# traveller59/spconv

Hardware: NVIDIA H100
Metric: active-voxels/sec fwd+bwd SubMConv3d 3^3 C=64 (higher is better)
Workload: dtype fp16

## Files before the change

### spconv_b200/csrc/common.cuh

```cuda
#pragma once
#include <cuda_runtime.h>
#include <cuda_fp16.h>
#include <cuda_bf16.h>
#include <stdint.h>
#include <stdio.h>
#include <string.h>
#include <stdarg.h>
#include <type_traits>

#include "../../include/spconv_b200.h"

namespace spx {

void set_error(const char *fmt, ...);
void count_launch(int n = 1);
void set_family(int f);
int sm_count();
int current_device();

struct RuntimeCfg {
    int force_simt = 0, force_tc = 0;
    bool tf32_dgrad_fma = false;
    bool tf32_wgrad_fma = false;
};
RuntimeCfg &runtime_cfg();

bool func_configured(const void *fn, int dev);

#define SPX_CHECK_CUDA(expr)                                                              \
    do {                                                                                  \
        cudaError_t _e = (expr);                                                          \
        if (_e != cudaSuccess) {                                                          \
            (void)cudaGetLastError();                                                     \
            spx::set_error("%s failed: %s (%s:%d)", #expr, cudaGetErrorString(_e),        \
                           __FILE__, __LINE__);                                           \
            return 1;                                                                     \
        }                                                                                 \
    } while (0)

#define SPX_CHECK_LAUNCH(name)                                                            \
    do {                                                                                  \
        cudaError_t _e = cudaGetLastError();                                              \
        if (_e != cudaSuccess) {                                                          \
            spx::set_error("launch of %s failed: %s (%s:%d)", name,                       \
                           cudaGetErrorString(_e), __FILE__, __LINE__);                   \
            return 1;                                                                     \
        }                                                                                 \
        spx::count_launch();                                                              \
    } while (0)

#define SPX_REQUIRE(cond, ...)                                                            \
    do {                                                                                  \
        if (!(cond)) {                                                                    \
            spx::set_error(__VA_ARGS__);                                                  \
            return 2;                                                                     \
        }                                                                                 \
    } while (0)

static inline size_t align_up(size_t x, size_t a) { return (x + a - 1) / a * a; }
static inline int64_t div_up64(int64_t a, int64_t b) { return (a + b - 1) / b; }

struct WorkspaceCarver {
    char *base;
    size_t off = 0, cap;
    WorkspaceCarver(void *p, size_t bytes) : base((char *)p), cap(bytes) {}
    template <typename T> T *take(size_t n) {
        off = align_up(off, 256);
        T *r = (T *)(base + off);
        off += n * sizeof(T);
        return r;
    }
    bool ok() const { return off <= cap; }
};

__host__ __device__ static inline int dtype_bytes(int dt) {
    switch (dt) {
        case SPX_F32: return 4;
        case SPX_F16: return 2;
        case SPX_BF16: return 2;
        case SPX_I8: return 1;
    }
    return 0;
}

#ifdef __CUDACC__

template <typename T> __device__ __forceinline__ float to_float(T v);
template <> __device__ __forceinline__ float to_float<float>(float v) { return v; }
template <> __device__ __forceinline__ float to_float<__half>(__half v) { return __half2float(v); }
template <> __device__ __forceinline__ float to_float<__nv_bfloat16>(__nv_bfloat16 v) { return __bfloat162float(v); }
template <> __device__ __forceinline__ float to_float<int8_t>(int8_t v) { return (float)v; }

template <typename T> __device__ __forceinline__ T from_float(float v);
template <> __device__ __forceinline__ float from_float<float>(float v) { return v; }
template <> __device__ __forceinline__ __half from_float<__half>(float v) { return __float2half_rn(v); }
template <> __device__ __forceinline__ __nv_bfloat16 from_float<__nv_bfloat16>(float v) { return __float2bfloat16_rn(v); }

__device__ __forceinline__ float apply_act(float v, int act, float alpha) {
    switch (act) {
        case SPX_ACT_RELU: return v > 0.f ? v : 0.f;
        case SPX_ACT_SIGMOID: return 1.f / (1.f + __expf(-v));
        case SPX_ACT_LEAKY_RELU: return v >= 0.f ? v : v * alpha;
        default: return v;
    }
}

__device__ __forceinline__ uint32_t smem_u32(const void *p) {
    return (uint32_t)__cvta_generic_to_shared(p);
}

__device__ __forceinline__ void mbar_init(uint64_t *bar, uint32_t count) {
    asm volatile("mbarrier.init.shared::cta.b64 [%0], %1;" ::"r"(smem_u32(bar)), "r"(count) : "memory");
}
__device__ __forceinline__ void mbar_fence_init() {
    asm volatile("fence.mbarrier_init.release.cluster;" ::: "memory");
}
__device__ __forceinline__ void mbar_arrive(uint64_t *bar) {
    asm volatile("{\n\t.reg .b64 st;\n\tmbarrier.arrive.shared::cta.b64 st, [%0];\n\t}" ::"r"(smem_u32(bar)) : "memory");
}
__device__ __forceinline__ void mbar_arrive_expect_tx(uint64_t *bar, uint32_t bytes) {
    asm volatile("{\n\t.reg .b64 st;\n\tmbarrier.arrive.expect_tx.shared::cta.b64 st, [%0], %1;\n\t}" ::"r"(smem_u32(bar)), "r"(bytes) : "memory");
}
__device__ __forceinline__ bool mbar_try_wait(uint64_t *bar, uint32_t parity) {
    uint32_t ok;
    asm volatile(
        "{\n\t.reg .pred p;\n\t"
        "mbarrier.try_wait.parity.shared::cta.b64 p, [%1], %2;\n\t"
        "selp.u32 %0, 1, 0, p;\n\t}"
        : "=r"(ok) : "r"(smem_u32(bar)), "r"(parity) : "memory");
    return ok != 0;
}
__device__ __forceinline__ void mbar_wait(uint64_t *bar, uint32_t parity) {
    if (mbar_try_wait(bar, parity)) return;
    const long long t0 = clock64();
    uint32_t spins = 0;
    while (!mbar_try_wait(bar, parity)) {
        if ((++spins & 0x3FFFu) == 0u && clock64() - t0 > 4000000000ll) {
            printf("spconv_b200: mbarrier wait timed out (block %d thread %d bar 0x%x parity %u)\n",
                   (int)blockIdx.x, (int)threadIdx.x, smem_u32(bar), parity);
            __trap();
        }
// ... 69 lines not shown
```

### spconv_b200/csrc/rulebook.cu

```cuda
#include "common.cuh"
#include "gemm.cuh"
#include "hash.cuh"
#include "rank.cuh"
#include <cub/cub.cuh>

namespace spx {
size_t radix_argsort_workspace_bytes(int64_t n);
int radix_argsort_pair(uint32_t *mask0, int32_t *argsort0, int64_t n0, uint32_t *mask1, int32_t *argsort1, int64_t n1,
                       int key_bits, void *ws0, size_t ws0_bytes, void *ws1, size_t ws1_bytes, cudaStream_t stream);
}

namespace spx {

struct Geom {
    int ndim, batch, kv;
    int in_dims[SPX_MAX_NDIM], out_dims[SPX_MAX_NDIM], ksize[SPX_MAX_NDIM];
    int stride[SPX_MAX_NDIM], padding[SPX_MAX_NDIM], dilation[SPX_MAX_NDIM];
    int transposed;
};

static Geom make_geom(const spx_conv_geometry *g, bool subm) {
    Geom r;
    memset(&r, 0, sizeof(r));
    r.ndim = g->ndim;
    r.batch = g->batch_size;
    r.kv = 1;
    r.transposed = g->transposed;
    for (int a = 0; a < g->ndim; ++a) {
        r.in_dims[a] = g->in_dims[a];
        r.ksize[a] = g->ksize[a];
        r.dilation[a] = g->dilation[a];
        r.kv *= g->ksize[a];
        if (subm) {
            r.out_dims[a] = g->in_dims[a];
            r.stride[a] = 1;
            r.padding[a] = (g->ksize[a] / 2) * g->dilation[a];
        } else {
            r.out_dims[a] = g->out_dims[a];
            r.stride[a] = g->stride[a];
            r.padding[a] = g->padding[a];
        }
    }
    return r;
}

static bool needs_i64(const Geom &g, const int *dims) {
    double v = (double)g.batch;
    for (int a = 0; a < g.ndim; ++a) v *= (double)dims[a];
    return v >= 2147483647.0;
}

__device__ __forceinline__ void load_coord(const int32_t *indices, int64_t i, int ndim, int (&c)[SPX_MAX_NDIM + 1]) {
    if (ndim == 3) {
        int4 v = __ldg(reinterpret_cast<const int4 *>(indices) + i);
        c[0] = v.x; c[1] = v.y; c[2] = v.z; c[3] = v.w;
    } else {
        const int32_t *p = indices + i * (ndim + 1);
#pragma unroll
        for (int a = 0; a <= SPX_MAX_NDIM; ++a) if (a <= ndim) c[a] = __ldg(p + a);
    }
}

__device__ __forceinline__ int64_t linear_key(const int (&c)[SPX_MAX_NDIM + 1], const int *dims, int ndim) {
    int64_t k = c[0];
#pragma unroll
    for (int a = 0; a < SPX_MAX_NDIM; ++a) if (a < ndim) k = k * dims[a] + c[a + 1];
    return k;
}

__device__ __forceinline__ void offset_taps(int k, const int *ksize, int ndim, int (&r)[SPX_MAX_NDIM]) {
#pragma unroll
    for (int a = SPX_MAX_NDIM - 1; a >= 0; --a) if (a < ndim) { r[a] = k % ksize[a]; k /= ksize[a]; }
}

template <typename Table>
__global__ void subm_insert_kernel(Table table, Geom g, const int32_t *__restrict__ indices, int64_t N) {
    int64_t i = blockIdx.x * (int64_t)blockDim.x + threadIdx.x;
    if (i >= N) return;
    int c[SPX_MAX_NDIM + 1];
    load_coord(indices, i, g.ndim, c);
    table.insert_min(linear_key(c, g.in_dims, g.ndim), (int32_t)i);
}

template <typename Table>
__global__ void subm_probe_kernel(Table table, Geom g, const int32_t *__restrict__ indices, int64_t N,
                                  int32_t *__restrict__ pair_fwd, int32_t *__restrict__ pair_bwd,
                                  uint32_t *__restrict__ mask, int words) {
    int64_t o = blockIdx.x * (int64_t)blockDim.x + threadIdx.x;
    if (o >= N) return;
    int c[SPX_MAX_NDIM + 1];
    load_coord(indices, o, g.ndim, c);
    const int kv = g.kv;
    uint32_t mword = 0;
    int r[SPX_MAX_NDIM] = {0, 0, 0, 0};
    for (int k = 0; k < kv; ++k) {
        int32_t found = -1;
        if (k == kv / 2) {
            found = (int32_t)o;
        } else {
            int q[SPX_MAX_NDIM + 1];
            q[0] = c[0];
            bool valid = c[0] >= 0 && c[0] < g.batch;
#pragma unroll
            for (int a = 0; a < SPX_MAX_NDIM; ++a) {
                if (a < g.ndim) {
                    q[a + 1] = c[a + 1] - g.padding[a] + r[a] * g.dilation[a];
                    valid = valid && q[a + 1] >= 0 && q[a + 1] < g.in_dims[a];
                }
            }
            if (valid) {
                int32_t v;
                if (table.find_slot(linear_key(q, g.in_dims, g.ndim), v) >= 0) found = v;
            }
        }
        pair_fwd[(int64_t)k * N + o] = found;
        if (pair_bwd) pair_bwd[(int64_t)(kv - 1 - k) * N + o] = found;
        if (found >= 0) mword |= 1u << (k & 31);
        if (mask && ((k & 31) == 31 || k == kv - 1)) {
            mask[o * words + (k >> 5)] = mword;
            mword = 0;
        }
#pragma unroll
        for (int a = SPX_MAX_NDIM - 1; a >= 0; --a) {
            if (a < g.ndim) {
                if (++r[a] < g.ksize[a]) break;
                r[a] = 0;
            }
        }
    }
}

constexpr int K3_VOX = 128;
constexpr int K3_PER_LANE = K3_VOX / 32;
__global__ void __launch_bounds__(27 * 32, 2)
subm_probe_k3_kernel(Table32 table, Geom g, const int32_t *__restrict__ indices, int64_t N,
                     int32_t *__restrict__ pair_fwd, int32_t *__restrict__ pair_bwd,
                     uint32_t *__restrict__ mask, int32_t *__restrict__ row_table) {
    __shared__ uint32_t hit_col[27][K3_PER_LANE];
    __shared__ int32_t row_stage[K3_VOX][27];
    const int lane = threadIdx.x & 31;
    const int k = threadIdx.x >> 5;
    const int rz = k / 9, ry = (k / 3) % 3, rx = k % 3;
    const int64_t vbase = blockIdx.x * (int64_t)K3_VOX;
    const int D0 = g.in_dims[0], D1 = g.in_dims[1], D2 = g.in_dims[2];
    const int oz = (rz - 1) * g.dilation[0], oy = (ry - 1) * g.dilation[1], ox = (rx - 1) * g.dilation[2];
    int4 c[K3_PER_LANE];
#pragma unroll
    for (int j = 0; j < K3_PER_LANE; ++j) {
        const int64_t o = vbase + j * 32 + lane;
        c[j] = o < N ? __ldg(reinterpret_cast<const int4 *>(indices) + o) : make_int4(-1, 0, 0, 0);
    }
    uint32_t key[K3_PER_LANE], h[K3_PER_LANE];
    unsigned long long cur[K3_PER_LANE];
    uint32_t pending = 0;
#pragma unroll
    for (int j = 0; j < K3_PER_LANE; ++j) {
        const int qz = c[j].y + oz, qy = c[j].z + oy, qx = c[j].w + ox;
        const bool valid = k != 13 && c[j].x >= 0 && c[j].x < g.batch && qz >= 0 && qz < D0 && qy >= 0 && qy < D1 &&
                           qx >= 0 && qx < D2;
        key[j] = (uint32_t)(((c[j].x * D0 + qz) * D1 + qy) * D2 + qx);
        h[j] = mix32(key[j]) & table.cap_mask;
        cur[j] = valid ? __ldg(&table.slots[h[j]]) : Table32::EMPTY;
    }
#pragma unroll
    for (int j = 0; j < K3_PER_LANE; ++j)
        if (cur[j] != Table32::EMPTY && (uint32_t)(cur[j] >> 32) != key[j]) pending |= 1u << j;
    while (pending) {
#pragma unroll
        for (int j = 0; j < K3_PER_LANE; ++j)
            if (pending & (1u << j)) { h[j] = (h[j] + 1) & table.cap_mask; cur[j] = __ldg(&table.slots[h[j]]); }
#pragma unroll
        for (int j = 0; j < K3_PER_LANE; ++j)
            if ((pending & (1u << j)) && (cur[j] == Table32::EMPTY || (uint32_t)(cur[j] >> 32) == key[j]))
                pending &= ~(1u << j);
    }
#pragma unroll
    for (int j = 0; j < K3_PER_LANE; ++j) {
        const int64_t o = vbase + j * 32 + lane;
        int32_t found = cur[j] != Table32::EMPTY ? (int32_t)(uint32_t)cur[j] : -1;
        if (k == 13 && o < N) found = (int32_t)o;
        if (o < N) {
            pair_fwd[(int64_t)k * N + o] = found;
            if (pair_bwd) pair_bwd[(int64_t)(26 - k) * N + o] = found;
        }
        const uint32_t hits = __ballot_sync(0xffffffffu, found >= 0);
        if (lane == 0) hit_col[k][j] = hits;
        row_stage[j * 32 + lane][k] = found;
    }
    __syncthreads();
    if (mask && threadIdx.x < K3_VOX && vbase + threadIdx.x < N) {
        const int v = threadIdx.x;
        uint32_t m = 0;
#pragma unroll
        for (int kk = 0; kk < 27; ++kk) m |= ((hit_col[kk][v >> 5] >> (v & 31)) & 1u) << kk;
        mask[vbase + v] = m;
    }
    if (row_table) {
        for (int e = threadIdx.x; e < K3_VOX * 32; e += 27 * 32) {
            const int v = e >> 5, kk = e & 31;
            if (vbase + v < N) row_table[(vbase + v) * 32 + kk] = kk < 27 ? row_stage[v][kk] : -1;
        }
    }
}

__device__ __forceinline__ bool conv_out_coord(const Geom &g, const int (&c)[SPX_MAX_NDIM + 1],
                                               const int (&r)[SPX_MAX_NDIM], int (&o)[SPX_MAX_NDIM + 1]) {
    bool valid = c[0] >= 0 && c[0] < g.batch;
    o[0] = c[0];
#pragma unroll
    for (int a = 0; a < SPX_MAX_NDIM; ++a) {
        if (a < g.ndim) {
            if (g.transposed) {
                o[a + 1] = c[a + 1] * g.stride[a] - g.padding[a] + r[a] * g.dilation[a];
                valid = valid && o[a + 1] >= 0 && o[a + 1] < g.out_dims[a];
            } else {
                int h = c[a + 1] + g.padding[a] - r[a] * g.dilation[a];
                o[a + 1] = h / g.stride[a];
                valid = valid && o[a + 1] >= 0 && o[a + 1] < g.out_dims[a] && (h % g.stride[a] == 0);
            }
        }
    }
    return valid;
}

struct Taps3 { int r0, r1, r2; };
__device__ __forceinline__ Taps3 block_taps3(const Geom &g, int k) {
    Taps3 t;
    t.r2 = k % g.ksize[2]; k /= g.ksize[2];
    t.r1 = k % g.ksize[1]; k /= g.ksize[1];
    t.r0 = k;
    return t;
}
__device__ __forceinline__ bool axis_out(int c, int pad, int r, int dil, int stride, int odim, int &o) {
    const int h = c + pad - r * dil;
    if (h < 0) return false;
    if (stride == 1) o = h;
    else if (stride == 2) { if (h & 1) return false; o = h >> 1; }
    else { o = h / stride; if (o * stride != h) return false; }
    return o < odim;
}
__device__ __forceinline__ bool conv3_out_key(const Geom &g, const int4 c, const Taps3 &t, int64_t &key) {
    int o0, o1, o2;
    if (c.x < 0 || c.x >= g.batch) return false;
    if (!axis_out(c.y, g.padding[0], t.r0, g.dilation[0], g.stride[0], g.out_dims[0], o0)) return false;
    if (!axis_out(c.z, g.padding[1], t.r1, g.dilation[1], g.stride[1], g.out_dims[1], o1)) return false;
    if (!axis_out(c.w, g.padding[2], t.r2, g.dilation[2], g.stride[2], g.out_dims[2], o2)) return false;
    key = (((int64_t)c.x * g.out_dims[0] + o0) * g.out_dims[1] + o1) * g.out_dims[2] + o2;
    return true;
}

struct Axis3 { int o[3]; };
__device__ __forceinline__ Axis3 axis_taps3(int c, int pad, int dil, int stride, int odim) {
    Axis3 a;
#pragma unroll
    for (int r = 0; r < 3; ++r) { int o; a.o[r] = axis_out(c, pad, r, dil, stride, odim, o) ? o : -1; }
    return a;
}

template <typename Table>
__global__ void conv_pairs_k3_kernel(Table table, Geom g, const int32_t *__restrict__ indices, int64_t N, int64_t M,
                                     int32_t *__restrict__ pair_fwd, int32_t *__restrict__ pair_bwd,
                                     uint32_t *__restrict__ mask_bwd, uint32_t *__restrict__ mask_fwd_or) {
    const int64_t i = blockIdx.x * (int64_t)blockDim.x + threadIdx.x;
    if (i >= N) return;
    const int4 c = __ldg(reinterpret_cast<const int4 *>(indices) + i);
    const bool bok = c.x >= 0 && c.x < g.batch;
    const Axis3 az = axis_taps3(c.y, g.padding[0], g.dilation[0], g.stride[0], g.out_dims[0]);
    const Axis3 ay = axis_taps3(c.z, g.padding[1], g.dilation[1], g.stride[1], g.out_dims[1]);
    const Axis3 ax = axis_taps3(c.w, g.padding[2], g.dilation[2], g.stride[2], g.out_dims[2]);
    uint32_t mword = 0;
#pragma unroll
    for (int r0 = 0; r0 < 3; ++r0) {
#pragma unroll
        for (int r1 = 0; r1 < 3; ++r1) {
#pragma unroll
            for (int r2 = 0; r2 < 3; ++r2) {
                const int k = (r0 * 3 + r1) * 3 + r2;
                int32_t out = -1;
// ... 575 lines not shown
    __syncthreads();
    for (int t0 = 0; t0 < tiles; t0 += TO_THREADS) {
        for (int i = tid; i < (TO_THREADS / 32) * TO_BUCKETS; i += TO_THREADS) (&wcnt[0][0])[i] = 0;
        __syncthreads();
        const int t = t0 + tid;
        const bool ok = t < tiles;
        uint32_t m[4] = {0, 0, 0, 0};
        const int c = ok ? load_mask(t, m) : TO_BUCKETS - 1;
        const unsigned peers = __match_any_sync(0xffffffffu, ok ? c : -1);
        const int rank = __popc(peers & ((1u << lane) - 1u));
        if (ok && rank == 0) wcnt[warp][c] = __popc(peers);
        __syncthreads();
        const int live_warps = min(TO_THREADS / 32, (tiles - t0 + 31) / 32);
        for (int b = tid; b < TO_BUCKETS; b += TO_THREADS) {
            int run = bucket_base[b];
            for (int w = 0; w < live_warps; ++w) { const int n = wcnt[w][b]; wcnt[w][b] = run; run += n; }
            bucket_base[b] = run;
        }
        __syncthreads();
        if (ok) {
            int32_t *r = rec + (int64_t)(wcnt[warp][c] + rank) * TT_REC_INTS;
            *reinterpret_cast<int4 *>(r) = make_int4(t, (int)m[0], (int)m[1], (int)m[2]);
            *reinterpret_cast<int4 *>(r + 4) = make_int4((int)m[3], 0, 0, 0);
        }
        __syncthreads();
    }
}

}

using namespace spx;

static int validate_geom(const spx_conv_geometry *g) {
    SPX_REQUIRE(g != nullptr, "geometry is NULL");
    SPX_REQUIRE(g->ndim >= 1 && g->ndim <= SPX_MAX_NDIM, "ndim must be in [1, %d], got %d", SPX_MAX_NDIM, g->ndim);
    SPX_REQUIRE(g->batch_size > 0, "batch_size must be positive");
    for (int a = 0; a < g->ndim; ++a) {
        SPX_REQUIRE(g->ksize[a] > 0 && g->dilation[a] > 0 && g->in_dims[a] > 0, "bad ksize/dilation/dims on axis %d", a);
    }
    return 0;
}

struct RbLayout {
    size_t table_bytes, table_vals_bytes;
    uint32_t capacity;
    bool i64;
};

static RbLayout rb_layout(const Geom &g, int64_t items, const int *dims, int factor = 4) {
    RbLayout L;
    L.i64 = needs_i64(g, dims);
    L.capacity = table_capacity(items, factor);
    L.table_bytes = (size_t)L.capacity * 8;
    L.table_vals_bytes = L.i64 ? (size_t)L.capacity * 4 : 0;
    return L;
}

extern "C" int64_t spx_conv_max_out(const spx_conv_geometry *g, int64_t num_in) {
    int64_t res = num_in, kv = 1;
    for (int i = 0; i < g->ndim; ++i) {
        kv *= g->ksize[i];
        if (g->ksize[i] > g->stride[i]) res *= (g->ksize[i] + g->stride[i] - 1) / g->stride[i];
    }
    if (g->transposed) res = kv * num_in;
    if (res > kv * num_in) res = kv * num_in;
    return res;
}

static size_t sort_pairs_temp_bytes(int64_t n) {
    cudaGetLastError();
    size_t bytes = 0;
    cudaError_t e = cub::DeviceRadixSort::SortPairs(nullptr, bytes, (const uint32_t *)nullptr, (uint32_t *)nullptr,
                                                    (const uint32_t *)nullptr, (uint32_t *)nullptr, (int)n);
    const size_t floor_bytes = (size_t)(n > 0 ? n : 1) * 16 + (1u << 20);
    if (e != cudaSuccess) { cudaGetLastError(); return floor_bytes; }
    return bytes > floor_bytes ? bytes : floor_bytes;
}

static bool subm_k3_path(const Geom &gg) {
    return !needs_i64(gg, gg.in_dims) && gg.ndim == 3 && gg.ksize[0] == 3 && gg.ksize[1] == 3 && gg.ksize[2] == 3;
}

static int subm_rulebook(const spx_conv_geometry *g, const int32_t *indices, int64_t N, int32_t *pair_fwd,
                         int32_t *pair_bwd, uint32_t *mask, int32_t *row_table, void *workspace,
                         size_t workspace_bytes, spx_stream_t stream_) {
    if (validate_geom(g)) return 2;
    for (int a = 0; a < g->ndim; ++a)
        SPX_REQUIRE(g->ksize[a] % 2 == 1, "subm only support odd ksize");
    SPX_REQUIRE(N >= 0 && N < 2147483647ll, "bad N");
    if (N == 0) return 0;
    SPX_REQUIRE(indices && pair_fwd && workspace, "NULL pointer argument");
    cudaStream_t stream = (cudaStream_t)stream_;
    Geom gg = make_geom(g, true);
    SPX_REQUIRE((int64_t)gg.kv * N < 2147483647ll * 4, "kv*N too large");
    RbLayout L = rb_layout(gg, N, gg.in_dims);
    WorkspaceCarver ws(workspace, workspace_bytes);
    void *tbl = ws.take<char>(L.table_bytes);
    int32_t *tvals = L.i64 ? ws.take<int32_t>(L.capacity) : nullptr;
    SPX_REQUIRE(ws.ok(), "rulebook workspace too small: need %zu, have %zu", ws.off, workspace_bytes);
    int words = (gg.kv + 31) / 32;
    const int T = 128;
    unsigned nblk = (unsigned)div_up64(N, T);
    SPX_CHECK_CUDA(cudaMemsetAsync(tbl, 0xFF, L.table_bytes, stream));
    if (!L.i64) {
        Table32 t{(unsigned long long *)tbl, L.capacity - 1};
        subm_insert_kernel<<<nblk, T, 0, stream>>>(t, gg, indices, N);
        SPX_CHECK_LAUNCH("subm_insert_kernel");
        if (subm_k3_path(gg)) {
            subm_probe_k3_kernel<<<(unsigned)div_up64(N, K3_VOX), 27 * 32, 0, stream>>>(t, gg, indices, N, pair_fwd,
                                                                                        pair_bwd, mask, row_table);
        } else {
            subm_probe_kernel<<<nblk, T, 0, stream>>>(t, gg, indices, N, pair_fwd, pair_bwd, mask, words);
        }
        SPX_CHECK_LAUNCH("subm_probe_kernel");
    } else {
        SPX_CHECK_CUDA(cudaMemsetAsync(tvals, 0x7F, (size_t)L.capacity * 4, stream));
        Table64 t{(long long *)tbl, tvals, L.capacity - 1};
        subm_insert_kernel<<<nblk, T, 0, stream>>>(t, gg, indices, N);
        SPX_CHECK_LAUNCH("subm_insert_kernel");
        subm_probe_kernel<<<nblk, T, 0, stream>>>(t, gg, indices, N, pair_fwd, pair_bwd, mask, words);
        SPX_CHECK_LAUNCH("subm_probe_kernel");
    }
    return 0;
}

extern "C" int spx_subm_rulebook(const spx_conv_geometry *g, const int32_t *indices, int64_t N, int32_t *pair_fwd,
                                 int32_t *pair_bwd, uint32_t *mask, void *workspace, size_t workspace_bytes,
                                 spx_stream_t stream) {
    return subm_rulebook(g, indices, N, pair_fwd, pair_bwd, mask, nullptr, workspace, workspace_bytes, stream);
}


namespace {
struct ConvWs {
    void *tbl; int32_t *tvals;
    uint32_t *slot;
    uint32_t *rank_bitmap; int *rank_tiles;
    size_t rank_bytes; int64_t rank_ntiles;
    int *counter;
    size_t bytes;
    RbLayout L;
};

struct ConvStage1Record { const void *ws; uint32_t capacity; };
thread_local ConvStage1Record g_stage1 = {nullptr, 0};

uint32_t optimistic_capacity(int64_t max_out, uint32_t full_capacity) {
    uint32_t cap = table_capacity((max_out + 3) / 4, 2);
    return cap < full_capacity ? cap : full_capacity;
}
int carve_conv_ws(const spx_conv_geometry *g, const Geom &gg, int64_t N, void *workspace, size_t bytes, ConvWs &w) {
    int64_t max_out = spx_conv_max_out(g, N);
    w.L = rb_layout(gg, max_out, gg.out_dims, 2);
    WorkspaceCarver ws(workspace, bytes);
    w.tbl = ws.take<char>(w.L.table_bytes);
    w.tvals = w.L.i64 ? ws.take<int32_t>(w.L.capacity) : nullptr;
    w.slot = ws.take<uint32_t>(max_out);
    w.rank_bytes = rank_scratch_bytes((int64_t)gg.kv * N, &w.rank_ntiles);
    w.rank_bitmap = (uint32_t *)ws.take<char>(w.rank_bytes);
    w.rank_tiles = (int *)(w.rank_bitmap + w.rank_ntiles * RANK_TILE_WORDS);
    w.counter = ws.take<int>(64);
    w.bytes = ws.off;
    SPX_REQUIRE(ws.ok(), "rulebook workspace too small: need %zu, have %zu", ws.off, bytes);
    return 0;
}
}

extern "C" size_t spx_rulebook_workspace_size(const spx_conv_geometry *g, int64_t num_in, int64_t max_out, int is_subm) {
    if (!g || g->ndim < 1 || g->ndim > SPX_MAX_NDIM) return 0;
    Geom gg = make_geom(g, is_subm != 0);
    size_t total = 256;
    if (is_subm) {
        RbLayout L = rb_layout(gg, num_in, gg.in_dims);
        total += align_up(L.table_bytes, 256) + align_up(L.table_vals_bytes, 256);
    } else {
        (void)max_out;
        ConvWs w;
        carve_conv_ws(g, gg, num_in, nullptr, SIZE_MAX, w);
        total += align_up(w.bytes, 256);
    }
    return total + 1024;
}

extern "C" int spx_conv_rulebook_stage1(const spx_conv_geometry *g, const int32_t *indices, int64_t N,
                                        int64_t *num_out_host, void *workspace, size_t workspace_bytes,
                                        spx_stream_t stream_) {
    if (validate_geom(g)) return 2;
    SPX_REQUIRE(num_out_host != nullptr, "num_out_host is NULL");
    *num_out_host = 0;
    if (N == 0) return 0;
    SPX_REQUIRE(indices && workspace, "NULL pointer argument");
    for (int a = 0; a < g->ndim; ++a)
        SPX_REQUIRE(g->stride[a] > 0 && g->out_dims[a] > 0, "bad stride/out_dims on axis %d", a);
    cudaStream_t stream = (cudaStream_t)stream_;
    Geom gg = make_geom(g, false);
    SPX_REQUIRE((int64_t)gg.kv * N < 2000000000ll, "kv*N must stay below 2e9 (kv=%d, N=%lld)", gg.kv, (long long)N);
    ConvWs w;
    if (carve_conv_ws(g, gg, N, workspace, workspace_bytes, w)) return 2;
    const int T = 128;
    dim3 grid((unsigned)div_up64(N, T), gg.kv);
    const bool fast3 = gg.ndim == 3 && !gg.transposed;
    const bool k3 = fast3 && gg.ksize[0] == 3 && gg.ksize[1] == 3 && gg.ksize[2] == 3;
    g_stage1 = {workspace, w.L.capacity};
    const int64_t max_out = spx_conv_max_out(g, N);
    int host_state[2] = {0, 0};
    uint32_t capacity = optimistic_capacity(max_out, w.L.capacity);
    for (int attempt = 0; attempt < 2; ++attempt) {
        const int64_t zero_vec = (int64_t)(((char *)(w.counter + 64) - (char *)w.rank_bitmap) / 16);
        conv_clear_kernel<<<sm_count() * 4, 256, 0, stream>>>((uint4 *)w.tbl, (int64_t)capacity / 2,
                                                              w.L.i64 ? (uint4 *)w.tvals : nullptr,
                                                              w.L.i64 ? (int64_t)capacity / 4 : 0,
                                                              (uint4 *)w.rank_bitmap, zero_vec);
// ... 179 lines not shown
        count_launch(3);
        int32_t *t = cur; cur = nxt; nxt = t;
    }
    SPX_CHECK_CUDA(cudaMemcpyAsync(argsort, cur, (size_t)N * 4, cudaMemcpyDeviceToDevice, stream));
    gather_rows_kernel<<<nblk, 256, 0, stream>>>(mask, argsort, N, words, rows_tmp);
    SPX_CHECK_LAUNCH("gather_rows_kernel");
    SPX_CHECK_CUDA(cudaMemcpyAsync(mask, rows_tmp, (size_t)N * words * 4, cudaMemcpyDeviceToDevice, stream));
    return 0;
}

extern "C" size_t spx_tile_table_elems(int64_t rows, int kv) {
    return (size_t)tt_total_elems(div_up64(rows > 0 ? rows : 1, 128), kv);
}

static int build_tile_table(const int32_t *pair, int64_t pair_stride, int kv, const int32_t *argsort,
                            const uint32_t *mask, int64_t rows, const int32_t *row_table, int32_t *table,
                            uint32_t *tile_mask, spx_stream_t stream_) {
    SPX_REQUIRE(kv >= 1 && kv <= 128, "build_tile_table: kernel volume %d not in [1,128]", kv);
    if (rows == 0) return 0;
    SPX_REQUIRE((pair || row_table) && table && tile_mask, "build_tile_table: NULL pointer argument");
    cudaStream_t stream = (cudaStream_t)stream_;
    int words = (kv + 31) / 32;
    if (row_table) {
        SPX_REQUIRE(kv <= 32, "build_tile_table: row_table holds at most 32 offsets per row, kv = %d", kv);
        SPX_REQUIRE(((uintptr_t)row_table & 15u) == 0, "build_tile_table: row_table must be 16-byte aligned");
        build_tile_table_rows_kernel<<<(unsigned)div_up64(rows, 128), 128 * TT_SPLIT, 0, stream>>>(
            row_table, kv, argsort, mask, rows, table, tile_mask);
        SPX_CHECK_LAUNCH("build_tile_table_rows_kernel");
    } else {
        TtJobs jobs;
        memset(&jobs, 0, sizeof(jobs));
        jobs.j[0] = TtJob{pair, pair_stride, argsort, mask, rows, table, tile_mask};
        build_tile_table_kernel<<<dim3((unsigned)div_up64(rows, 128), 1), 128 * TT_SPLIT, 0, stream>>>(jobs, kv, words);
        SPX_CHECK_LAUNCH("build_tile_table_kernel");
    }
    const int64_t tiles = div_up64(rows, 128);
    SPX_REQUIRE(tiles < 2147483647ll, "build_tile_table: too many tiles");
    SPX_REQUIRE(((uintptr_t)table & 15u) == 0, "build_tile_table: table must be 16-byte aligned");
    int32_t *rec = table + tt_blocks_elems(tiles, kv);
    ToJobs oj;
    memset(&oj, 0, sizeof(oj));
    oj.j[0] = ToJob{tile_mask, (int)tiles, rec, rec + tiles * TT_REC_INTS};
    tile_order_kernel<<<1, TO_THREADS, 0, stream>>>(oj, words);
    SPX_CHECK_LAUNCH("tile_order_kernel");
    return 0;
}

extern "C" int spx_build_tile_table(const int32_t *pair, int64_t pair_stride, int kv, const int32_t *argsort,
                                    const uint32_t *mask, int64_t rows, int32_t *table, uint32_t *tile_mask,
                                    spx_stream_t stream) {
    return build_tile_table(pair, pair_stride, kv, argsort, mask, rows, nullptr, table, tile_mask, stream);
}

static int build_tile_tables_pair(int kv, const int32_t *pair0, const int32_t *argsort0, const uint32_t *mask0, int64_t rows0,
                                  int32_t *table0, uint32_t *tmask0, const int32_t *pair1, const int32_t *argsort1,
                                  const uint32_t *mask1, int64_t rows1, int32_t *table1, uint32_t *tmask1,
                                  cudaStream_t stream) {
    SPX_REQUIRE(kv >= 1 && kv <= 128, "build_tile_table: kernel volume %d not in [1,128]", kv);
    const int words = (kv + 31) / 32;
    const int64_t tiles0 = div_up64(rows0, 128), tiles1 = div_up64(rows1, 128);
    SPX_REQUIRE(tiles0 < 2147483647ll && tiles1 < 2147483647ll, "build_tile_table: too many tiles");
    SPX_REQUIRE((((uintptr_t)table0 | (uintptr_t)table1) & 15u) == 0, "build_tile_table: table must be 16-byte aligned");
    TtJobs jobs;
    memset(&jobs, 0, sizeof(jobs));
    jobs.j[0] = TtJob{pair0, rows0, argsort0, mask0, rows0, table0, tmask0};
    jobs.j[1] = TtJob{pair1, rows1, argsort1, mask1, rows1, table1, tmask1};
    const int64_t tmax = tiles0 > tiles1 ? tiles0 : tiles1;
    build_tile_table_kernel<<<dim3((unsigned)tmax, 2), 128 * TT_SPLIT, 0, stream>>>(jobs, kv, words);
    SPX_CHECK_LAUNCH("build_tile_table_kernel");
    int32_t *rec0 = table0 + tt_blocks_elems(tiles0, kv), *rec1 = table1 + tt_blocks_elems(tiles1, kv);
    ToJobs oj;
    memset(&oj, 0, sizeof(oj));
    oj.j[0] = ToJob{tmask0, (int)tiles0, rec0, rec0 + tiles0 * TT_REC_INTS};
    oj.j[1] = ToJob{tmask1, (int)tiles1, rec1, rec1 + tiles1 * TT_REC_INTS};
    tile_order_kernel<<<2, TO_THREADS, 0, stream>>>(oj, words);
    SPX_CHECK_LAUNCH("tile_order_kernel");
    return 0;
}


static size_t subm_row_table_bytes(const spx_conv_geometry *g, int64_t N) {
    return subm_k3_path(make_geom(g, true)) ? align_up((size_t)N * 32 * sizeof(int32_t), 256) : 0;
}

extern "C" size_t spx_subm_rulebook_all_workspace_size(const spx_conv_geometry *g, int64_t N) {
    if (!g || g->ndim < 1 || g->ndim > SPX_MAX_NDIM) return 0;
    int kv = 1;
    for (int a = 0; a < g->ndim; ++a) kv *= g->ksize[a];
    const size_t a = spx_rulebook_workspace_size(g, N, 0, 1);
    const size_t b = spx_mask_argsort_workspace_size(N, (kv + 31) / 32);
    return align_up(a > b ? a : b, 256) + subm_row_table_bytes(g, N) + 256;
}

extern "C" int spx_subm_rulebook_all(const spx_conv_geometry *g, const int32_t *indices, int64_t N, int32_t *pair_fwd,
                                     int32_t *pair_bwd, uint32_t *mask, int32_t *argsort, int do_sort,
                                     int32_t *tile_table, uint32_t *tile_mask, void *workspace, size_t workspace_bytes,
                                     spx_stream_t stream) {
    if (validate_geom(g)) return 2;
    if (N == 0) return 0;
    SPX_REQUIRE(mask && argsort && tile_table && tile_mask && workspace, "subm_rulebook_all: NULL pointer argument");
    SPX_REQUIRE(workspace_bytes >= spx_subm_rulebook_all_workspace_size(g, N), "subm_rulebook_all: workspace too small");
    int kv = 1;
    for (int a = 0; a < g->ndim; ++a) kv *= g->ksize[a];
    const int words = (kv + 31) / 32;
    const size_t rb = spx_rulebook_workspace_size(g, N, 0, 1), as = spx_mask_argsort_workspace_size(N, words);
    const size_t shared = align_up(rb > as ? rb : as, 256);
    int32_t *row_table = subm_row_table_bytes(g, N) ? (int32_t *)((char *)workspace + shared) : nullptr;
    if (int rc = subm_rulebook(g, indices, N, pair_fwd, pair_bwd, mask, row_table, workspace, rb, stream)) return rc;
    if (int rc = spx_mask_argsort(mask, argsort, N, words, kv, do_sort, workspace, as, stream)) return rc;
    return build_tile_table(pair_fwd, N, kv, argsort, mask, N, row_table, tile_table, tile_mask, stream);
}

static int conv_sort_and_tiles(int kv, int64_t N, int64_t M, int32_t *pair_fwd, int32_t *pair_bwd, uint32_t *mask_fwd,
                               uint32_t *mask_bwd, int32_t *argsort_fwd, int32_t *argsort_bwd, int do_sort,
                               int32_t *table_fwd, uint32_t *tmask_fwd, int32_t *table_bwd, uint32_t *tmask_bwd,
                               void *sort_ws, size_t sort_bytes, spx_stream_t stream) {
    const int words = (kv + 31) / 32;
    const bool train = argsort_bwd != nullptr;
    if (words == 1 && do_sort && train) {
        const size_t half = (sort_bytes / 2) & ~(size_t)255;
        const int key_bits = kv < 32 ? kv : 32;
        if (int rc = radix_argsort_pair(mask_fwd, argsort_fwd, M, mask_bwd, argsort_bwd, N, key_bits, sort_ws, half,
                                        (char *)sort_ws + half, half, (cudaStream_t)stream)) return rc;
        return build_tile_tables_pair(kv, pair_fwd, argsort_fwd, mask_fwd, M, table_fwd, tmask_fwd, pair_bwd, argsort_bwd,
                                      mask_bwd, N, table_bwd, tmask_bwd, (cudaStream_t)stream);
    }
    if (int rc = spx_mask_argsort(mask_fwd, argsort_fwd, M, words, kv, do_sort, sort_ws, sort_bytes, stream)) return rc;
    if (int rc = spx_build_tile_table(pair_fwd, M, kv, argsort_fwd, mask_fwd, M, table_fwd, tmask_fwd, stream)) return rc;
    if (!train) return 0;
    if (int rc = spx_mask_argsort(mask_bwd, argsort_bwd, N, words, kv, do_sort, sort_ws, sort_bytes, stream)) return rc;
    return spx_build_tile_table(pair_bwd, N, kv, argsort_bwd, mask_bwd, N, table_bwd, tmask_bwd, stream);
}

extern "C" size_t spx_conv_rulebook_all_workspace_size(const spx_conv_geometry *g, int64_t N) {
    if (!g || g->ndim < 1 || g->ndim > SPX_MAX_NDIM) return 0;
    int kv = 1;
    for (int a = 0; a < g->ndim; ++a) kv *= g->ksize[a];
    const int64_t max_rows = spx_conv_max_out(g, N) > N ? spx_conv_max_out(g, N) : N;
    return align_up(spx_rulebook_workspace_size(g, N, 0, 0), 256) +
           2 * align_up(spx_mask_argsort_workspace_size(max_rows, (kv + 31) / 32), 256) + 256;
}

extern "C" int spx_conv_rulebook_stage2_all(const spx_conv_geometry *g, const int32_t *indices, int64_t N, int64_t M,
                                            int32_t *out_inds, int32_t *pair_fwd, int32_t *pair_bwd, uint32_t *mask_fwd,
                                            uint32_t *mask_bwd, int32_t *argsort_fwd, int32_t *argsort_bwd, int do_sort,
                                            int32_t *table_fwd, uint32_t *tmask_fwd, int32_t *table_bwd,
                                            uint32_t *tmask_bwd, void *workspace, size_t workspace_bytes,
                                            spx_stream_t stream) {
    if (validate_geom(g)) return 2;
    if (N == 0 || M == 0) return 0;
    SPX_REQUIRE(mask_fwd && mask_bwd && argsort_fwd && table_fwd && tmask_fwd && workspace,
                "conv_rulebook_stage2_all: NULL pointer argument");
    const bool train = argsort_bwd != nullptr;
    SPX_REQUIRE((table_bwd != nullptr) == train && (tmask_bwd != nullptr) == train,
                "conv_rulebook_stage2_all: argsort_bwd, table_bwd and tmask_bwd must all be given (training) or all be "
                "NULL (inference)");
    SPX_REQUIRE(workspace_bytes >= spx_conv_rulebook_all_workspace_size(g, N), "conv_rulebook_stage2_all: workspace too small");
    int kv = 1;
    for (int a = 0; a < g->ndim; ++a) kv *= g->ksize[a];
    const size_t rb = spx_rulebook_workspace_size(g, N, 0, 0);
    void *sort_ws = (char *)workspace + align_up(rb, 256);
    const size_t sort_bytes = workspace_bytes - align_up(rb, 256);
    if (int rc = spx_conv_rulebook_stage2(g, indices, N, M, out_inds, pair_fwd, pair_bwd, mask_fwd, mask_bwd, workspace, rb, stream)) return rc;
    return conv_sort_and_tiles(kv, N, M, pair_fwd, pair_bwd, mask_fwd, mask_bwd, argsort_fwd, argsort_bwd, do_sort,
                               table_fwd, tmask_fwd, table_bwd, tmask_bwd, sort_ws, sort_bytes, stream);
}

namespace {
struct BoundedWs {
    void *tbl; int32_t *tvals;
    uint32_t *rank_bitmap; int *rank_tiles; int64_t rank_ntiles;
    int *state;
    void *sort_ws; size_t sort_bytes;
    size_t bytes;
    RbLayout L;
};

void carve_bounded_ws(const Geom &gg, int64_t N, int64_t bound, void *workspace, size_t bytes, BoundedWs &w) {
    w.L = rb_layout(gg, bound, gg.out_dims, 2);
    WorkspaceCarver ws(workspace, bytes);
    w.tbl = ws.take<char>(w.L.table_bytes);
    w.tvals = w.L.i64 ? ws.take<int32_t>(w.L.capacity) : nullptr;
    const size_t rank_bytes = rank_scratch_bytes((int64_t)gg.kv * N, &w.rank_ntiles);
    w.rank_bitmap = (uint32_t *)ws.take<char>(rank_bytes);
    w.rank_tiles = (int *)(w.rank_bitmap + w.rank_ntiles * RANK_TILE_WORDS);
    w.state = ws.take<int>(64);
    const int64_t max_rows = bound > N ? bound : N;
    w.sort_bytes = 2 * align_up(spx_mask_argsort_workspace_size(max_rows, (gg.kv + 31) / 32), 256);
    w.sort_ws = ws.take<char>(w.sort_bytes);
    w.bytes = ws.off;
}

// ... 115 lines not shown
```

### spconv_b200/csrc/sort.cu

```cuda
#include "common.cuh"

namespace spx {

constexpr int RS_BITS = 9;
constexpr int RS_BINS = 1 << RS_BITS;
constexpr int RS_THREADS = 256;
constexpr int RS_WARPS = RS_THREADS / 32;
constexpr int RS_ITEMS = 4;
constexpr int RS_TILE = RS_THREADS * RS_ITEMS;
constexpr int RS_AGG_BITS = 11;
constexpr int RS_AGG_SLOTS = 1 << RS_AGG_BITS;
constexpr int RS_TILE_SHIFT = 10;
static_assert((1 << RS_TILE_SHIFT) == RS_TILE, "tile shift");

struct RsJob {
    const uint32_t *kin; const int32_t *vin;
    int64_t n; int nblk;
    int *counts; int *totals;
    uint32_t *kout; int32_t *vout;
    int *counts_next;
};
struct RsJobs { RsJob j[2]; };

__global__ void __launch_bounds__(RS_THREADS)
rs_hist_kernel(const RsJobs jobs, int shift) {
    const RsJob &J = jobs.j[blockIdx.y];
    if ((int)blockIdx.x >= J.nblk) return;
    const uint32_t *__restrict__ keys = J.kin;
    const int64_t n = J.n;
    const int nblk = J.nblk;
    int *__restrict__ counts = J.counts;
    __shared__ int hist[RS_BINS];
    for (int i = threadIdx.x; i < RS_BINS; i += RS_THREADS) hist[i] = 0;
    __syncthreads();
    const int64_t base = (int64_t)blockIdx.x * RS_TILE;
#pragma unroll
    for (int j = 0; j < RS_ITEMS; ++j) {
        const int64_t i = base + j * RS_THREADS + threadIdx.x;
        if (i < n) atomicAdd(&hist[(keys[i] >> shift) & (RS_BINS - 1)], 1);
    }
    __syncthreads();
    for (int d = threadIdx.x; d < RS_BINS; d += RS_THREADS) counts[(int64_t)d * nblk + blockIdx.x] = hist[d];
}

__global__ void __launch_bounds__(RS_THREADS)
rs_scan_kernel(const RsJobs jobs) {
    const RsJob &J = jobs.j[blockIdx.y];
    int *__restrict__ counts = J.counts;
    const int nblk = J.nblk;
    int *__restrict__ totals = J.totals;
    int *__restrict__ clear_next = J.counts_next;
    if (nblk == 0) return;
    const int d = blockIdx.x;
    if (clear_next)
        for (int b = threadIdx.x; b < nblk; b += RS_THREADS) clear_next[(int64_t)d * nblk + b] = 0;
    __shared__ int warp_sums[RS_WARPS];
    __shared__ int carry_s;
    if (threadIdx.x == 0) carry_s = 0;
    __syncthreads();
    const int lane = threadIdx.x & 31, warp = threadIdx.x >> 5;
    for (int b0 = 0; b0 < nblk; b0 += RS_THREADS) {
        const int b = b0 + threadIdx.x;
        const int v = b < nblk ? counts[(int64_t)d * nblk + b] : 0;
        int incl = v;
#pragma unroll
        for (int o = 1; o < 32; o <<= 1) {
            int t = __shfl_up_sync(0xffffffffu, incl, o);
            if (lane >= o) incl += t;
        }
        if (lane == 31) warp_sums[warp] = incl;
        __syncthreads();
        int wbase = 0;
        for (int w = 0; w < warp; ++w) wbase += warp_sums[w];
        const int carry = carry_s;
        if (b < nblk) counts[(int64_t)d * nblk + b] = carry + wbase + incl - v;
        __syncthreads();
        if (threadIdx.x == RS_THREADS - 1) carry_s = carry + wbase + incl;
        __syncthreads();
    }
    if (threadIdx.x == 0) totals[d] = carry_s;
}

template <bool IOTA_IN>
__global__ void __launch_bounds__(RS_THREADS)
rs_scatter_kernel(const RsJobs jobs, int shift) {
    const RsJob &J = jobs.j[blockIdx.y];
    if ((int)blockIdx.x >= J.nblk) return;
    const uint32_t *__restrict__ keys_in = J.kin;
    const int32_t *__restrict__ vals_in = J.vin;
    const int64_t n = J.n;
    const int nblk = J.nblk;
    const int *__restrict__ counts = J.counts;
    const int *__restrict__ totals = J.totals;
    uint32_t *__restrict__ keys_out = J.kout;
    int32_t *__restrict__ vals_out = J.vout;
// ... 30 lines not shown
        digit_base[q * RS_THREADS + tid] = run + wbase + incl - v + my_before[q];
        run += all;
        __syncthreads();
    }

    const int64_t tile_base = (int64_t)blk * RS_TILE + warp * (32 * RS_ITEMS);
    uint32_t key[RS_ITEMS];
    int32_t val[RS_ITEMS];
    int rank[RS_ITEMS];
#pragma unroll
    for (int r = 0; r < RS_ITEMS; ++r) {
        const int64_t i = tile_base + r * 32 + lane;
        const bool ok = i < n;
        key[r] = ok ? keys_in[i] : 0xffffffffu;
        val[r] = ok ? (IOTA_IN ? (int32_t)i : vals_in[i]) : -1;
        const int d = ok ? (int)((key[r] >> shift) & (RS_BINS - 1)) : RS_BINS;
        const unsigned peers = __match_any_sync(0xffffffffu, d);
        const int leader = __ffs(peers) - 1;
        int old = 0;
        if (ok && lane == leader) { old = warp_cnt[warp][d]; warp_cnt[warp][d] = old + __popc(peers); }
        old = __shfl_sync(0xffffffffu, old, leader);
        rank[r] = old + __popc(peers & ((1u << lane) - 1u));
        __syncwarp();
    }
    __syncthreads();
    for (int d = tid; d < RS_BINS; d += RS_THREADS) {
        int acc = 0;
#pragma unroll
        for (int w = 0; w < RS_WARPS; ++w) { const int c = warp_cnt[w][d]; warp_cnt[w][d] = acc; acc += c; }
    }
    __syncthreads();
#pragma unroll
    for (int r = 0; r < RS_ITEMS; ++r) {
        const int64_t i = tile_base + r * 32 + lane;
        if (i < n) {
            const int d = (int)((key[r] >> shift) & (RS_BINS - 1));
            const int pos = digit_base[d] + warp_cnt[warp][d] + rank[r];
            keys_out[pos] = key[r];
            vals_out[pos] = val[r];
            if (counts_next) {
                const int dn = (int)((key[r] >> (shift + RS_BITS)) & (RS_BINS - 1));
                const int cell = dn * nblk + (pos >> RS_TILE_SHIFT);
                uint32_t slot = ((uint32_t)cell * 2654435761u) >> (32 - RS_AGG_BITS);
                while (true) {
                    const int prev = atomicCAS(&agg_cell[slot], -1, cell);
                    if (prev == -1 || prev == cell) { atomicAdd(&agg_cnt[slot], 1); break; }
                    slot = (slot + 1) & (RS_AGG_SLOTS - 1);
                }
            }
        }
    }
    if (counts_next) {
        __syncthreads();
        for (int s2 = tid; s2 < RS_AGG_SLOTS; s2 += RS_THREADS)
            if (agg_cell[s2] >= 0) atomicAdd(counts_next + agg_cell[s2], agg_cnt[s2]);
    }
}

size_t radix_argsort_workspace_bytes(int64_t n) {
    const int64_t nblk = div_up64(n > 0 ? n : 1, RS_TILE);
    return 4 * align_up((size_t)n * 4, 256) + 2 * align_up((size_t)RS_BINS * nblk * 4, 256) +
           align_up(RS_BINS * 4, 256) + 1024;
}

namespace {
struct RsPlan {
    uint32_t *keys_a, *keys_b; int32_t *vals_a, *vals_b;
    int *counts_ab[2]; int *totals;
    int nblk;
};
int rs_carve(int64_t n, void *workspace, size_t bytes, RsPlan &p) {
    WorkspaceCarver ws(workspace, bytes);
    p.keys_a = ws.take<uint32_t>(n); p.vals_a = ws.take<int32_t>(n);
    p.keys_b = ws.take<uint32_t>(n); p.vals_b = ws.take<int32_t>(n);
    p.nblk = (int)div_up64(n, RS_TILE);
    p.counts_ab[0] = ws.take<int>((size_t)RS_BINS * p.nblk);
    p.counts_ab[1] = ws.take<int>((size_t)RS_BINS * p.nblk);
    p.totals = ws.take<int>(RS_BINS);
    SPX_REQUIRE(ws.ok(), "argsort workspace too small: need %zu, have %zu", ws.off, bytes);
    return 0;
}
}

int radix_argsort_pair(uint32_t *mask0, int32_t *argsort0, int64_t n0, uint32_t *mask1, int32_t *argsort1, int64_t n1,
                       int key_bits, void *ws0, size_t ws0_bytes, void *ws1, size_t ws1_bytes, cudaStream_t stream) {
    if (n0 == 0 && n1 == 0) return 0;
    if (n0 == 0) return radix_argsort_pair(mask1, argsort1, n1, nullptr, nullptr, 0, key_bits, ws1, ws1_bytes, nullptr, 0, stream);
    if (key_bits < 1) key_bits = 1;
    if (key_bits > 32) key_bits = 32;
    const int passes = (key_bits + RS_BITS - 1) / RS_BITS;
    const int njobs = n1 > 0 ? 2 : 1;
    RsPlan pl[2];
    uint32_t *masks[2] = {mask0, mask1};
    int32_t *argsorts[2] = {argsort0, argsort1};
    const int64_t ns[2] = {n0, n1};
    if (int rc = rs_carve(n0, ws0, ws0_bytes, pl[0])) return rc;
    if (njobs == 2) if (int rc = rs_carve(n1, ws1, ws1_bytes, pl[1])) return rc;
    RsJobs jobs;
    memset(&jobs, 0, sizeof(jobs));
    int max_nblk = 0;
    for (int q = 0; q < njobs; ++q) {
        jobs.j[q].kin = masks[q]; jobs.j[q].vin = nullptr; jobs.j[q].n = ns[q]; jobs.j[q].nblk = pl[q].nblk;
        jobs.j[q].totals = pl[q].totals;
        if (pl[q].nblk > max_nblk) max_nblk = pl[q].nblk;
    }
    const dim3 grid_tiles(max_nblk, njobs), grid_scan(RS_BINS, njobs);
    for (int q = 0; q < njobs; ++q) jobs.j[q].counts = pl[q].counts_ab[0];
    rs_hist_kernel<<<grid_tiles, RS_THREADS, 0, stream>>>(jobs, 0);
    SPX_CHECK_LAUNCH("rs_hist_kernel");
    for (int pass = 0; pass < passes; ++pass) {
        const bool last = pass == passes - 1;
        for (int q = 0; q < njobs; ++q) {
            RsJob &J = jobs.j[q];
            J.kout = (pass & 1) ? pl[q].keys_b : pl[q].keys_a;
            J.vout = (pass & 1) ? pl[q].vals_b : pl[q].vals_a;
            if (last && pass > 0) { J.kout = masks[q]; J.vout = argsorts[q]; }
            J.counts = pl[q].counts_ab[pass & 1];
            J.counts_next = last ? nullptr : pl[q].counts_ab[(pass + 1) & 1];
        }
        rs_scan_kernel<<<grid_scan, RS_THREADS, 0, stream>>>(jobs);
        SPX_CHECK_LAUNCH("rs_scan_kernel");
        if (pass == 0) rs_scatter_kernel<true><<<grid_tiles, RS_THREADS, 0, stream>>>(jobs, pass * RS_BITS);
        else rs_scatter_kernel<false><<<grid_tiles, RS_THREADS, 0, stream>>>(jobs, pass * RS_BITS);
        SPX_CHECK_LAUNCH("rs_scatter_kernel");
        for (int q = 0; q < njobs; ++q) { jobs.j[q].kin = jobs.j[q].kout; jobs.j[q].vin = jobs.j[q].vout; }
    }
    if (passes == 1) {
        for (int q = 0; q < njobs; ++q) {
            SPX_CHECK_CUDA(cudaMemcpyAsync(masks[q], pl[q].keys_a, (size_t)ns[q] * 4, cudaMemcpyDeviceToDevice, stream));
            SPX_CHECK_CUDA(cudaMemcpyAsync(argsorts[q], pl[q].vals_a, (size_t)ns[q] * 4, cudaMemcpyDeviceToDevice, stream));
        }
    }
    return 0;
}

}
```

Before: 522.5 million.

## Fuse first radix-sort digit histogram into the 3x3x3 subm probe kernel

The 3x3x3 submanifold probe kernel now counts the low 9-bit digit of each voxel mask in shared memory and atomically adds the counts into a per-sort-tile histogram. The histogram is zeroed inside the hash insert kernel. The argsort can then skip its first histogram kernel launch and the extra read of the mask array. The cost is shared-memory atomics and global atomics in the probe, plus extra workspace for the histogram.

New measurement: 511.7 million, median of 6. -2.1%, worse.

```diff
diff --git a/spconv_b200/csrc/common.cuh b/spconv_b200/csrc/common.cuh
--- a/spconv_b200/csrc/common.cuh
+++ b/spconv_b200/csrc/common.cuh
@@ -57,6 +57,10 @@
         }                                                                                 \
     } while (0)
 
+constexpr int RS_BITS = 9;
+constexpr int RS_BINS = 1 << RS_BITS;
+constexpr int RS_TILE_SHIFT = 10;
+
 static inline size_t align_up(size_t x, size_t a) { return (x + a - 1) / a * a; }
 static inline int64_t div_up64(int64_t a, int64_t b) { return (a + b - 1) / b; }
 
diff --git a/spconv_b200/csrc/rulebook.cu b/spconv_b200/csrc/rulebook.cu
--- a/spconv_b200/csrc/rulebook.cu
+++ b/spconv_b200/csrc/rulebook.cu
@@ -8,6 +8,9 @@
 size_t radix_argsort_workspace_bytes(int64_t n);
 int radix_argsort_pair(uint32_t *mask0, int32_t *argsort0, int64_t n0, uint32_t *mask1, int32_t *argsort1, int64_t n1,
                        int key_bits, void *ws0, size_t ws0_bytes, void *ws1, size_t ws1_bytes, cudaStream_t stream);
+size_t radix_hist_bytes(int64_t n);
+int radix_argsort_hist(uint32_t *mask, int32_t *argsort, int64_t n, int key_bits, int *hist0, void *ws, size_t ws_bytes,
+                       cudaStream_t stream);
 }
 
 namespace spx {
@@ -74,8 +77,10 @@
 }
 
 template <typename Table>
-__global__ void subm_insert_kernel(Table table, Geom g, const int32_t *__restrict__ indices, int64_t N) {
+__global__ void subm_insert_kernel(Table table, Geom g, const int32_t *__restrict__ indices, int64_t N,
+                                   int *__restrict__ zero = nullptr, int64_t zero_n = 0) {
     int64_t i = blockIdx.x * (int64_t)blockDim.x + threadIdx.x;
+    for (int64_t z = i; z < zero_n; z += (int64_t)gridDim.x * blockDim.x) zero[z] = 0;
     if (i >= N) return;
     int c[SPX_MAX_NDIM + 1];
     load_coord(indices, i, g.ndim, c);
@@ -132,12 +137,17 @@
 
 constexpr int K3_VOX = 128;
 constexpr int K3_PER_LANE = K3_VOX / 32;
+static_assert(((1 << RS_TILE_SHIFT) % K3_VOX) == 0, "a probe block must lie in one sort block");
 __global__ void __launch_bounds__(27 * 32, 2)
 subm_probe_k3_kernel(Table32 table, Geom g, const int32_t *__restrict__ indices, int64_t N,
                      int32_t *__restrict__ pair_fwd, int32_t *__restrict__ pair_bwd,
-                     uint32_t *__restrict__ mask, int32_t *__restrict__ row_table) {
+                     uint32_t *__restrict__ mask, int32_t *__restrict__ row_table, int *__restrict__ hist0,
+                     int sort_blocks) {
     __shared__ uint32_t hit_col[27][K3_PER_LANE];
     __shared__ int32_t row_stage[K3_VOX][27];
+    __shared__ int digit_cnt[RS_BINS];
+    if (hist0)
+        for (int d = threadIdx.x; d < RS_BINS; d += 27 * 32) digit_cnt[d] = 0;
     const int lane = threadIdx.x & 31;
     const int k = threadIdx.x >> 5;
     const int rz = k / 9, ry = (k / 3) % 3, rx = k % 3;
@@ -194,6 +204,13 @@
 #pragma unroll
         for (int kk = 0; kk < 27; ++kk) m |= ((hit_col[kk][v >> 5] >> (v & 31)) & 1u) << kk;
         mask[vbase + v] = m;
+        if (hist0) atomicAdd(&digit_cnt[m & (RS_BINS - 1)], 1);
+    }
+    if (hist0) {
+        __syncthreads();
+        const int64_t sb = vbase >> RS_TILE_SHIFT;
+        for (int d = threadIdx.x; d < RS_BINS; d += 27 * 32)
+            if (digit_cnt[d]) atomicAdd(hist0 + (int64_t)d * sort_blocks + sb, digit_cnt[d]);
     }
     if (row_table) {
         for (int e = threadIdx.x; e < K3_VOX * 32; e += 27 * 32) {
@@ -935,7 +952,7 @@
 }
 
 static int subm_rulebook(const spx_conv_geometry *g, const int32_t *indices, int64_t N, int32_t *pair_fwd,
-                         int32_t *pair_bwd, uint32_t *mask, int32_t *row_table, void *workspace,
+                         int32_t *pair_bwd, uint32_t *mask, int32_t *row_table, int *hist0, void *workspace,
                          size_t workspace_bytes, spx_stream_t stream_) {
     if (validate_geom(g)) return 2;
     for (int a = 0; a < g->ndim; ++a)
@@ -957,11 +974,15 @@
     SPX_CHECK_CUDA(cudaMemsetAsync(tbl, 0xFF, L.table_bytes, stream));
     if (!L.i64) {
         Table32 t{(unsigned long long *)tbl, L.capacity - 1};
-        subm_insert_kernel<<<nblk, T, 0, stream>>>(t, gg, indices, N);
+        const bool k3 = subm_k3_path(gg);
+        SPX_REQUIRE(!hist0 || (k3 && mask), "subm_rulebook: the sort histogram needs the 3x3x3 probe and the mask");
+        const int sort_blocks = (int)div_up64(N, 1 << RS_TILE_SHIFT);
+        subm_insert_kernel<<<nblk, T, 0, stream>>>(t, gg, indices, N, hist0, hist0 ? (int64_t)RS_BINS * sort_blocks : 0);
         SPX_CHECK_LAUNCH("subm_insert_kernel");
-        if (subm_k3_path(gg)) {
+        if (k3) {
             subm_probe_k3_kernel<<<(unsigned)div_up64(N, K3_VOX), 27 * 32, 0, stream>>>(t, gg, indices, N, pair_fwd,
-                                                                                        pair_bwd, mask, row_table);
+                                                                                        pair_bwd, mask, row_table, hist0,
+                                                                                        sort_blocks);
         } else {
             subm_probe_kernel<<<nblk, T, 0, stream>>>(t, gg, indices, N, pair_fwd, pair_bwd, mask, words);
         }
@@ -980,7 +1001,7 @@
 extern "C" int spx_subm_rulebook(const spx_conv_geometry *g, const int32_t *indices, int64_t N, int32_t *pair_fwd,
                                  int32_t *pair_bwd, uint32_t *mask, void *workspace, size_t workspace_bytes,
                                  spx_stream_t stream) {
-    return subm_rulebook(g, indices, N, pair_fwd, pair_bwd, mask, nullptr, workspace, workspace_bytes, stream);
+    return subm_rulebook(g, indices, N, pair_fwd, pair_bwd, mask, nullptr, nullptr, workspace, workspace_bytes, stream);
 }
 
 
@@ -1326,6 +1347,9 @@
 static size_t subm_row_table_bytes(const spx_conv_geometry *g, int64_t N) {
     return subm_k3_path(make_geom(g, true)) ? align_up((size_t)N * 32 * sizeof(int32_t), 256) : 0;
 }
+static size_t subm_hist_bytes(const spx_conv_geometry *g, int64_t N) {
+    return subm_k3_path(make_geom(g, true)) ? align_up(radix_hist_bytes(N), 256) : 0;
+}
 
 extern "C" size_t spx_subm_rulebook_all_workspace_size(const spx_conv_geometry *g, int64_t N) {
     if (!g || g->ndim < 1 || g->ndim > SPX_MAX_NDIM) return 0;
@@ -1333,7 +1357,7 @@
     for (int a = 0; a < g->ndim; ++a) kv *= g->ksize[a];
     const size_t a = spx_rulebook_workspace_size(g, N, 0, 1);
     const size_t b = spx_mask_argsort_workspace_size(N, (kv + 31) / 32);
-    return align_up(a > b ? a : b, 256) + subm_row_table_bytes(g, N) + 256;
+    return align_up(a > b ? a : b, 256) + subm_row_table_bytes(g, N) + subm_hist_bytes(g, N) + 256;
 }
 
 extern "C" int spx_subm_rulebook_all(const spx_conv_geometry *g, const int32_t *indices, int64_t N, int32_t *pair_fwd,
@@ -1349,9 +1373,15 @@
     const int words = (kv + 31) / 32;
     const size_t rb = spx_rulebook_workspace_size(g, N, 0, 1), as = spx_mask_argsort_workspace_size(N, words);
     const size_t shared = align_up(rb > as ? rb : as, 256);
-    int32_t *row_table = subm_row_table_bytes(g, N) ? (int32_t *)((char *)workspace + shared) : nullptr;
-    if (int rc = subm_rulebook(g, indices, N, pair_fwd, pair_bwd, mask, row_table, workspace, rb, stream)) return rc;
-    if (int rc = spx_mask_argsort(mask, argsort, N, words, kv, do_sort, workspace, as, stream)) return rc;
+    const size_t row_bytes = subm_row_table_bytes(g, N);
+    int32_t *row_table = row_bytes ? (int32_t *)((char *)workspace + shared) : nullptr;
+    int *hist0 = subm_hist_bytes(g, N) && do_sort ? (int *)((char *)workspace + shared + row_bytes) : nullptr;
+    if (int rc = subm_rulebook(g, indices, N, pair_fwd, pair_bwd, mask, row_table, hist0, workspace, rb, stream)) return rc;
+    if (hist0) {
+        if (int rc = radix_argsort_hist(mask, argsort, N, kv, hist0, workspace, as, (cudaStream_t)stream)) return rc;
+    } else if (int rc = spx_mask_argsort(mask, argsort, N, words, kv, do_sort, workspace, as, stream)) {
+        return rc;
+    }
     return build_tile_table(pair_fwd, N, kv, argsort, mask, N, row_table, tile_table, tile_mask, stream);
 }
 
diff --git a/spconv_b200/csrc/sort.cu b/spconv_b200/csrc/sort.cu
--- a/spconv_b200/csrc/sort.cu
+++ b/spconv_b200/csrc/sort.cu
@@ -2,15 +2,12 @@
 
 namespace spx {
 
-constexpr int RS_BITS = 9;
-constexpr int RS_BINS = 1 << RS_BITS;
 constexpr int RS_THREADS = 256;
 constexpr int RS_WARPS = RS_THREADS / 32;
 constexpr int RS_ITEMS = 4;
 constexpr int RS_TILE = RS_THREADS * RS_ITEMS;
 constexpr int RS_AGG_BITS = 11;
 constexpr int RS_AGG_SLOTS = 1 << RS_AGG_BITS;
-constexpr int RS_TILE_SHIFT = 10;
 static_assert((1 << RS_TILE_SHIFT) == RS_TILE, "tile shift");
 
 struct RsJob {
@@ -207,10 +204,14 @@
 }
 }
 
-int radix_argsort_pair(uint32_t *mask0, int32_t *argsort0, int64_t n0, uint32_t *mask1, int32_t *argsort1, int64_t n1,
-                       int key_bits, void *ws0, size_t ws0_bytes, void *ws1, size_t ws1_bytes, cudaStream_t stream) {
+size_t radix_hist_bytes(int64_t n) { return (size_t)RS_BINS * div_up64(n > 0 ? n : 1, RS_TILE) * sizeof(int); }
+
+static int radix_argsort_impl(uint32_t *mask0, int32_t *argsort0, int64_t n0, uint32_t *mask1, int32_t *argsort1,
+                              int64_t n1, int key_bits, void *ws0, size_t ws0_bytes, void *ws1, size_t ws1_bytes,
+                              int *hist0, cudaStream_t stream) {
     if (n0 == 0 && n1 == 0) return 0;
-    if (n0 == 0) return radix_argsort_pair(mask1, argsort1, n1, nullptr, nullptr, 0, key_bits, ws1, ws1_bytes, nullptr, 0, stream);
+    if (n0 == 0) return radix_argsort_impl(mask1, argsort1, n1, nullptr, nullptr, 0, key_bits, ws1, ws1_bytes, nullptr, 0,
+                                           nullptr, stream);
     if (key_bits < 1) key_bits = 1;
     if (key_bits > 32) key_bits = 32;
     const int passes = (key_bits + RS_BITS - 1) / RS_BITS;
@@ -221,6 +222,8 @@
     const int64_t ns[2] = {n0, n1};
     if (int rc = rs_carve(n0, ws0, ws0_bytes, pl[0])) return rc;
     if (njobs == 2) if (int rc = rs_carve(n1, ws1, ws1_bytes, pl[1])) return rc;
+    SPX_REQUIRE(!hist0 || njobs == 1, "radix argsort: a precomputed histogram serves one job only");
+    if (hist0) pl[0].counts_ab[0] = hist0;
     RsJobs jobs;
     memset(&jobs, 0, sizeof(jobs));
     int max_nblk = 0;
@@ -231,8 +234,10 @@
     }
     const dim3 grid_tiles(max_nblk, njobs), grid_scan(RS_BINS, njobs);
     for (int q = 0; q < njobs; ++q) jobs.j[q].counts = pl[q].counts_ab[0];
-    rs_hist_kernel<<<grid_tiles, RS_THREADS, 0, stream>>>(jobs, 0);
-    SPX_CHECK_LAUNCH("rs_hist_kernel");
+    if (!hist0) {
+        rs_hist_kernel<<<grid_tiles, RS_THREADS, 0, stream>>>(jobs, 0);
+        SPX_CHECK_LAUNCH("rs_hist_kernel");
+    }
     for (int pass = 0; pass < passes; ++pass) {
         const bool last = pass == passes - 1;
         for (int q = 0; q < njobs; ++q) {
@@ -259,4 +264,15 @@
     return 0;
 }
 
-}
+int radix_argsort_pair(uint32_t *mask0, int32_t *argsort0, int64_t n0, uint32_t *mask1, int32_t *argsort1, int64_t n1,
+                       int key_bits, void *ws0, size_t ws0_bytes, void *ws1, size_t ws1_bytes, cudaStream_t stream) {
+    return radix_argsort_impl(mask0, argsort0, n0, mask1, argsort1, n1, key_bits, ws0, ws0_bytes, ws1, ws1_bytes, nullptr,
+                              stream);
+}
+
+int radix_argsort_hist(uint32_t *mask, int32_t *argsort, int64_t n, int key_bits, int *hist0, void *ws, size_t ws_bytes,
+                       cudaStream_t stream) {
+    return radix_argsort_impl(mask, argsort, n, nullptr, nullptr, 0, key_bits, ws, ws_bytes, nullptr, 0, hist0, stream);
+}
+
+}
```
